# merijn-23/magr-ray-tracer

Measured on AMD Instinct MI355X. Metric: Mrays/sec + extend-kernel HBM GB/s, sponza 1080p 256spp, higher is better.
Workload: dtype f32

## Files before the change

### include/rt355.h

```cpp
#ifndef RT355_H
#define RT355_H
#include "rt355_types.h"

#ifdef __cplusplus
extern "C" {
#endif

#define RT_OK            0
#define RT_E_INVALID    (-1)
#define RT_E_DEVICE     (-2)
#define RT_E_NOMEM      (-3)
#define RT_E_UNSUPPORTED (-4)

#define RT_SHADING_SIMPLE       0
#define RT_SHADING_NEE          1
#define RT_SAMPLING_HEMISPHERE  0
#define RT_SAMPLING_COSINE      1
#define RT_ACCEL_BVH2           0
#define RT_ACCEL_BVH4           1

typedef struct RtCtx RtCtx;

typedef struct RtConfig {
    int32_t width, height;
// ... 21 lines not shown
    uint64_t shadow_rays;
    uint64_t frames;
    uint64_t extend_node_issues, extend_leaf_issues, connect_node_issues, connect_leaf_issues;
    uint64_t extend_loop_node_events, extend_loop_leaf_events, connect_loop_node_events, connect_loop_leaf_events;
} RtCounters;

typedef struct RtStageTimes {
    double  generate_ms, extend_ms, shade_ms, compact_ms, connect_ms, accumulate_ms;
    int64_t generate_launches, extend_launches, shade_launches, compact_launches, connect_launches, accumulate_launches;
} RtStageTimes;

typedef struct RtKernelInfo {
    int32_t layout;
    int32_t persist, persist4;
    int32_t stack_entries;
    int32_t persist_grid, persist_grid_connect, shade_grid;
    int32_t n_blas;
} RtKernelInfo;

const char* rt_last_error(void);
int rt_device_count(void);
int rt_kernel_info(RtCtx* ctx, RtKernelInfo* out);
int rt_builtins(RtCtx* ctx);

int rt_create(const RtConfig* cfg, RtCtx** out);
int rt_destroy(RtCtx* ctx);

int rt_upload_scene(RtCtx* ctx,
                    const RtPrimitive* prims, int32_t nPrims,
                    const RtMaterial* mats, int32_t nMats,
                    const RtFloat4* textures, int32_t nTexels,
                    const uint32_t* lights, int32_t nLights,
                    const void* bvhNodes, int32_t nNodes,
                    const uint32_t* primIdx, int32_t nIdx,
                    const RtTLASNode* tlas, int32_t nTlas,
                    const RtBVHInstance* blas, int32_t nBlas);

int rt_upload_scene_bvh2(RtCtx* ctx,
                         const RtPrimitive* prims, int32_t nPrims, const RtMaterial* mats, int32_t nMats,
                         const RtFloat4* textures, int32_t nTexels, const uint32_t* lights, int32_t nLights,
                         const RtBVHNode2* bvhNodes, int32_t nNodes, const uint32_t* primIdx, int32_t nIdx,
                         const RtTLASNode* tlas, int32_t nTlas, const RtBVHInstance* blas, int32_t nBlas);

int rt_validate_scene(int32_t accel,
                      const RtPrimitive* prims, int32_t nPrims, const RtMaterial* mats, int32_t nMats,
                      const RtFloat4* textures, int32_t nTexels, const uint32_t* lights, int32_t nLights,
// ... 151 lines not shown
```

### magr_ray_tracer_amd/_lib.py

```python
import ctypes as C
import os

import numpy as np

_PKG = os.path.dirname(os.path.abspath(__file__))

f4 = np.dtype((np.float32, 4))
Ray = np.dtype([("O", f4), ("D", f4), ("rD", f4), ("N", f4), ("I", f4), ("intensity", f4), ("t", "<f4"),
                ("primIdx", "<i4"), ("bounces", "<i4"), ("pixelIdx", "<i4"), ("inside", "u1"), ("lastSpecular", "u1"),
                ("_pad0", "u1", 2), ("u", "<f4"), ("v", "<f4"), ("_pad1", "<u4")], align=False)
ShadowRay = np.dtype([("I", f4), ("L", f4), ("Nl", f4), ("intensity", f4), ("BRDF", f4), ("lightIdx", "<i4"),
                      ("pixelIdx", "<i4"), ("dotNL", "<f4"), ("dist", "<f4")])
Material = np.dtype([("color", f4), ("absorption", f4), ("specular", "<f4"), ("n1", "<f4"), ("n2", "<f4"),
                     ("isDielectric", "u1"), ("_pad0", "u1", 3), ("texIdx", "<i4"), ("texW", "<i4"), ("texH", "<i4"),
                     ("isLight", "u1"), ("_pad1", "u1", 3), ("emittance", f4)])
Primitive = np.dtype([("v0", f4), ("v1", f4), ("v2", f4), ("N", f4), ("centroid", f4), ("uv0", "<f4", 2), ("uv1", "<f4", 2),
                      ("uv2", "<f4", 2), ("_padt", "<f4", 2), ("objType", "<i4"), ("matIdx", "<i4"), ("area", "<f4"),
                      ("_pad", "<u4")])
Camera = np.dtype([("type", "<i4"), ("fov", "<f4"), ("aperture", "<f4"), ("focalLength", "<f4"), ("forward", f4),
                   ("right", f4), ("up", f4), ("origin", f4), ("horizontal", f4), ("vertical", f4), ("topLeft", f4)])
Settings = np.dtype([("numPrimitives", "<i4"), ("numLights", "<i4"), ("tracerType", "<i4"), ("frames", "<i4"),
                     ("antiAliasing", "<i4"), ("numInRays", "<i4"), ("numOutRays", "<i4"), ("shadowRays", "<i4"),
                     ("renderBVH", "<i4"), ("focalLength", "<f4")])
BVHNode2 = np.dtype([("aabbMin", f4), ("aabbMax", f4), ("first", "<u4"), ("count", "<u4"), ("_pad", "<u4", 2)])
# ... 43 lines not shown


def builtins_value(name):
    try:
        return BUILTINS[name]
    except (KeyError, TypeError):
        raise ValueError(f"builtins must be None, 'ieee' or 'reference', not {name!r}") from None


RT_OK, RT_E_INVALID, RT_E_DEVICE, RT_E_NOMEM, RT_E_UNSUPPORTED = 0, -1, -2, -3, -4
SCENE_ARRAYS = {"prims": 0, "bvh": 1, "tlas": 2, "instances": 3, "pairs": 4, "triRecs": 5, "shadeRecs": 6, "lightRecs": 7,
                "tlasPairs": 8, "tlasPairsP": 9, "instRecs": 10}
SCENE_ARRAYS_BVH4 = {"quads": 11, "rootEntry": 12, "bvh2Kept": 13}
UpdateStats = np.dtype([("gpu_ms", "<f8"), ("prims", "<i4"), ("nodes", "<i4"), ("tlas_nodes", "<i4"), ("tlas_depth", "<i4"),
                        ("reconfigured", "<i4"), ("reserved", "<i4", 3)])
assert UpdateStats.itemsize == 40
REBUILD_SAH, REBUILD_LBVH, REBUILD_SBVH = 0, 1, 2
RebuildStats = np.dtype([(n, "<f8") for n in ("gpu_ms", "wall_ms", "stage_ms", "build_ms", "derive_ms", "tlas_ms", "commit_ms")] +
                        [(n, "<i4") for n in ("prims", "blas_built", "nodes", "n_idx", "max_depth", "tlas_nodes", "tlas_depth", "reconfigured")] +
                        [("spatial_splits", "<i4"), ("prims_clipped", "<i4")])
assert RebuildStats.itemsize == 96

DEVICE_SYMBOLS = [
    "rt_last_error", "rt_device_count", "rt_kernel_info", "rt_builtins", "rt_create", "rt_destroy", "rt_upload_scene", "rt_share_scene", "rt_set_seeds", "rt_seed_default",
    "rt_get_seeds", "rt_bind_accum", "rt_accum_device_ptr", "rt_stream", "rt_reset", "rt_render", "rt_synchronize", "rt_focus",
    "rt_read_accum", "rt_write_accum", "rt_postproc", "rt_read_counters", "rt_reset_counters", "rt_read_stage_times", "rt_reset_stage_times", "rt_set_profile",
    "rt_stage_begin_frame", "rt_stage_generate", "rt_stage_extend", "rt_stage_shade", "rt_stage_connect",
    "rt_debug_get_rays", "rt_debug_set_rays", "rt_debug_get_shadow", "rt_debug_enable_steps", "rt_debug_get_steps", "rt_debug_math",
    "rt_debug_math_sweep", "rt_debug_math_mode", "rt_debug_math_sweep_mode", "rt_validate_scene", "rt_build_bvh2", "rt_build_bvh2_sah", "rt_debug_sah_phases", "rt_build_bvh2_sbvh", "rt_debug_sbvh_phases", "rt_update_scene", "rt_group_update_scene", "rt_debug_get_scene_array",
    "rt_rebuild_scene", "rt_group_rebuild_scene", "rt_blas_ranges", "rt_debug_rebuild_allocations",
    "rt_build_bvh4", "rt_upload_scene_bvh2", "rt_group_upload_scene_bvh2",
    "rt_group_create", "rt_group_destroy", "rt_group_lanes", "rt_group_concurrency", "rt_group_lane", "rt_group_frames", "rt_group_upload_scene", "rt_group_share_scene",
    "rt_group_seed", "rt_group_reset", "rt_group_render", "rt_group_synchronize", "rt_group_sum", "rt_group_read_accum", "rt_group_focus",
    "rt_group_postproc"]
HOST_SYMBOLS = [
    "rth_last_error", "rth_scene_create", "rth_scene_destroy", "rth_add_material", "rth_add_texture", "rth_load_texture", "rth_add_sphere",
    "rth_add_plane", "rth_add_triangle", "rth_add_quad", "rth_add_triangles", "rth_build_blas", "rth_build_bvh4",
    "rth_build_tlas", "rth_bvh4_from_nodes", "rth_set_instance_transform", "rth_primitives", "rth_materials", "rth_textures", "rth_lights",
    "rth_bvh2_nodes", "rth_bvh4_nodes", "rth_prim_idx", "rth_tlas_nodes", "rth_blas_nodes", "rth_bvh_stats", "rth_camera",
    "rth_renderer_create", "rth_renderer_destroy", "rth_renderer_init", "rth_renderer_set_camera", "rth_renderer_tick",
    "rth_renderer_read", "rth_renderer_camera", "rth_seed_stream", "rth_load_model", "rth_save_png",
    "rth_set_build_threads", "rth_renderer_save_frame", "rth_renderer_camera_move", "rth_renderer_camera_mouse", "rth_renderer_camera_zoom", "rth_renderer_frames", "rth_renderer_set_lanes", "rth_renderer_set_builtins", "rth_renderer_builtins",
    "rth_build_blas_lbvh", "rth_build_bvh2_lbvh", "rth_lbvh_stats", "rth_set_primitives", "rth_refit",
    "rth_build_blas_sah_gpu", "rth_build_bvh2_sah", "rth_build_blas_sbvh_gpu", "rth_build_bvh2_sbvh", "rth_rebuild", "rth_blas_ranges",
    "rth_build_bvh4_gpu", "rth_build_bvh4_levels"]

_dev = None
# ... 18 lines not shown

def device_lib(variant=None):
    global _dev
    if variant:
        if variant not in _variants:
            keep, _dev = _dev, None
            try:
                _variants[variant] = _bind_device(_load(f"librt355_{variant}.so", local=True))
            finally:
                _dev = keep
        return _variants[variant]
    if _dev is None:
        _dev = _bind_device(_load("librt355.so"))
    return _dev


def _bind_device(lib):
    if True:
        vp, i32, i64 = C.c_void_p, C.c_int32, C.c_int64
        lib.rt_last_error.restype = C.c_char_p
        lib.rt_create.argtypes = [vp, C.POINTER(vp)]
        lib.rt_kernel_info.argtypes = [vp, vp]
        lib.rt_builtins.argtypes = [vp]
        lib.rt_destroy.argtypes = [vp]
        lib.rt_upload_scene.argtypes = [vp, vp, i32, vp, i32, vp, i32, vp, i32, vp, i32, vp, i32, vp, i32, vp, i32]
        lib.rt_upload_scene_bvh2.argtypes = lib.rt_upload_scene.argtypes
        lib.rt_group_upload_scene_bvh2.argtypes = lib.rt_upload_scene.argtypes
        lib.rt_build_bvh4.argtypes = [i32, vp, i32, i32, vp, i32, vp, vp]
        lib.rt_share_scene.argtypes = [vp, vp]
        lib.rt_set_seeds.argtypes = [vp, vp, i64]
        lib.rt_seed_default.argtypes = [vp]
        lib.rt_get_seeds.argtypes = [vp, vp, i64]
        lib.rt_bind_accum.argtypes = [vp, vp]
        lib.rt_accum_device_ptr.argtypes = [vp]
        lib.rt_accum_device_ptr.restype = vp
        lib.rt_stream.argtypes = [vp]
        lib.rt_stream.restype = vp
        lib.rt_reset.argtypes = [vp]
        lib.rt_render.argtypes = [vp, vp, vp, i32]
        lib.rt_synchronize.argtypes = [vp]
        lib.rt_focus.argtypes = [vp, i32, i32, vp, C.POINTER(C.c_float)]
        lib.rt_read_accum.argtypes = [vp, vp]
        lib.rt_read_counters.argtypes = [vp, vp]
        lib.rt_write_accum.argtypes = [vp, vp]
        lib.rt_postproc.argtypes = [vp, i32, C.c_float, C.c_float, C.c_float, vp, vp]
        lib.rt_reset_counters.argtypes = [vp]
# ... 130 lines not shown
```

### magr_ray_tracer_amd/csrc/rt355.hip

```cpp
#include <hip/hip_runtime.h>
#include <hip/hip_ext.h>
#include <algorithm>
#include <chrono>
#include <cstdio>
#include <cmath>
#include <cstdlib>
#include <cstring>
#include <memory>
#include <atomic>
#include <string>
#include <vector>
#include "../../include/rt355.h"
#include "rt355_kernels.h"
#include "scene_dev.h"

using namespace rt355dev;
using namespace scenedev;

static constexpr int kAdmitAnySgpr = 6, kAdmit96Sgpr = 7;
static constexpr int kFitSeven = 22, kBackupWords = 10, kSpillCap = kFitSeven - kBackupWords;
static thread_local std::string g_err;
int rt355_set_error(int code, const char* msg) { g_err = msg; return code; }

struct RtCtx {
    RtConfig cfg{};
    hipStream_t stream = nullptr;
    hipStream_t home = nullptr;
    bool queued = true;
    DevScene sc{};
    DevQueues q{};
    DevVariant var{};
    int nPix = 0, firstPixel = 0, gridMax = 0;
    bool sceneLoaded = false, ownAccum = true;
    std::shared_ptr<SceneBag> scene;
    uint64_t sceneGen = 0;
    bool singleBlas = false;
    std::vector<void*> queueAllocs;
    float* dFocus = nullptr;
    RtRay* dRayIO = nullptr;
    uint64_t frames = 0, primaryRays = 0;
    struct Ev { hipEvent_t a, b; int stage; };
    std::vector<Ev> evPool; size_t evUsed = 0;
// ... 58 lines not shown
static bool bvh4_tlas_trav(const RtCtx* c) { return c->trav == TRAV_BVH4_TLAS || c->trav == TRAV_BVH4_TLAS_SPILL; }
static bool tlas_trav(const RtCtx* c) { return c->trav == TRAV_TLAS || c->trav == TRAV_TLAS_SPILL || bvh4_tlas_trav(c); }

extern "C" const char* rt_last_error(void) { return g_err.c_str(); }
extern "C" int rt_device_count(void) { int n = 0; if (hipGetDeviceCount(&n) != hipSuccess) return 0; return n; }
static int sync_scene_config(RtCtx* ctx);
extern "C" int rt_builtins(RtCtx* ctx)
{
    if (!ctx) return fail(RT_E_INVALID, "rt_builtins: null context");
    return ctx->cfg.builtins;
}
extern "C" int rt_kernel_info(RtCtx* ctx, RtKernelInfo* out)
{
    if (!ctx || !out) return fail(RT_E_INVALID, "rt_kernel_info: null argument");
    if (!ctx->sceneLoaded) return fail(RT_E_INVALID, "rt_kernel_info: no scene uploaded");
    if (const int rc = sync_scene_config(ctx)) return rc;
    const int persist = ctx->trav <= TRAV_TLAS_SPILL ? ctx->trav : 0;
    const int persist4 = ctx->trav == TRAV_BVH4 ? 1 : (ctx->trav == TRAV_BVH4_TLAS ? 2 : (ctx->trav == TRAV_BVH4_TLAS_SPILL ? 3 : 0));
    *out = RtKernelInfo{ ctx->layout, persist, persist4, spill_trav(ctx) ? ctx->spillCap : ctx->stackEntries, ctx->persistGrid, ctx->persistGridConnect,
                         ctx->shadeGrid, ctx->sc.nBlas };
    return RT_OK;
}

static void free_bag(std::vector<void*>& bag) { for (void* p : bag) (void)hipFree(p); bag.clear(); }

static void scene_release(RtCtx* ctx)
{
    if (!ctx->scene) return;
    auto& h = ctx->scene->holders;
    h.erase(std::remove(h.begin(), h.end(), ctx), h.end());
    ctx->scene.reset();
}
static void scene_hold(RtCtx* ctx, const std::shared_ptr<SceneBag>& bag)
{
    scene_release(ctx);
    ctx->scene = bag;
    bag->holders.push_back(ctx);
}
int SceneBag::wait_holders() const
{
    for (const RtCtx* h : holders) {
        HIPCHK(hipStreamSynchronize(h->stream));
        if (h->home != h->stream) HIPCHK(hipStreamSynchronize(h->home));
    }
    return RT_OK;
}

static size_t stack_bytes(const RtCtx* c) { return (size_t)c->stackEntries * kBlock * sizeof(uint32_t); }
static int tlas_stack_entries(const RtCtx* c) { return c->stackEntries + c->tlasDepth + 1; }
static int tlas_lds_entries(const RtCtx* c) { return spill_trav(c) ? c->spillCap : tlas_stack_entries(c); }
static size_t tlas_column_bytes(int entries) { return (size_t)(entries + kBackupWords) * kBlock * sizeof(uint32_t); }
static size_t tlas_stack_bytes(const RtCtx* c) { return tlas_column_bytes(tlas_lds_entries(c)); }
static inline dim3 grid_for(int n) { return dim3((unsigned)std::max(1, (n + kBlock - 1) / kBlock)); }

using PersistKernel = void (*)(DevScene, DevQueues, int, int, int, PersistTune);
using NestedKernel = void (*)(DevScene, DevQueues, int, int);
struct TraceLaunch {
    PersistKernel persist = nullptr;
    NestedKernel nested = nullptr;
    dim3 grid;
    size_t lds = 0;
    PersistTune tune{};
};
static TraceLaunch trace_launch(const RtCtx* c, int stage, int bounce, bool steps, int rays)
{
    TraceLaunch L;
    L.grid = grid_for(rays);
    L.lds = stack_bytes(c);
    const bool connect = stage == ST_CONNECT;
    const bool bvh4 = c->cfg.accel == RT_ACCEL_BVH4, l1 = c->layout == 1;
    switch (c->trav) {
    case TRAV_NESTED:
        if (connect) L.nested = bvh4 ? (l1 ? k_connect<RT_ACCEL_BVH4, 1> : k_connect<RT_ACCEL_BVH4, 0>) : (l1 ? k_connect<RT_ACCEL_BVH2, 1> : k_connect<RT_ACCEL_BVH2, 0>);
        else L.nested = bvh4 ? (l1 ? k_extend<RT_ACCEL_BVH4, 1> : k_extend<RT_ACCEL_BVH4, 0>) : (l1 ? k_extend<RT_ACCEL_BVH2, 1> : k_extend<RT_ACCEL_BVH2, 0>);
        break;
    case TRAV_BVH2:
        L.tune = connect ? c->tuneConnect : c->tune;
        if (connect) { L.persist = k_trace_persist<true>; L.grid = dim3(c->persistGridConnect); }
        else if (bounce > 0 || c->cfg.extend_variant == 3) { L.persist = steps ? k_trace_persist<false, false, true> : k_trace_persist<false>; L.grid = dim3(c->persistGrid); }
        else if (c->cfg.extend_variant == 5) L.nested = k_extend<RT_ACCEL_BVH2, 1>;
        else L.persist = c->coherent ? k_trace_persist<false, true> : (steps ? k_trace_persist<false, false, true> : k_trace_persist<false>);
        break;
    case TRAV_BVH4:
        L.tune = connect ? c->tuneConnect : c->tune4;
        L.persist = connect ? k_trace_persist4<true> : k_trace_persist4<false>;
        if (connect || bounce > 0) L.grid = dim3(connect ? c->persistGridConnect : c->persistGrid);
        break;
    case TRAV_TLAS:
    case TRAV_TLAS_SPILL: {
        const bool spill = c->trav == TRAV_TLAS_SPILL;
        L.lds = tlas_stack_bytes(c);
        if (connect) {
            L.tune = c->tuneConnect;
            L.persist = spill ? k_trace_persist_tlas<true, false, true> : k_trace_persist_tlas<true>;
            L.grid = dim3(c->persistGridConnect);
            break;
        }
        L.tune = c->tune;
        if (bounce > 0 || spill) L.grid = dim3(c->persistGrid);
        const bool coh = c->coherent && (bounce == 0 || c->coherent == 2) && (c->tune.flat || !spill);
        if (steps) L.persist = spill ? k_trace_persist_tlas<false, true, true> : k_trace_persist_tlas<false, true>;
        else if (coh) L.persist = spill ? k_trace_persist_tlas<false, false, true, true> : k_trace_persist_tlas<false, false, false, true>;
        else L.persist = spill ? k_trace_persist_tlas<false, false, true> : k_trace_persist_tlas<false>;
        break;
    }
    case TRAV_BVH4_TLAS:
    case TRAV_BVH4_TLAS_SPILL: {
        const bool spill = c->trav == TRAV_BVH4_TLAS_SPILL;
        L.lds = tlas_stack_bytes(c);
        if (connect) {
            L.tune = c->tuneConnect;
            L.persist = spill ? k_trace_persist4_tlas<true, false, true> : k_trace_persist4_tlas<true>;
            L.grid = dim3(c->persistGridConnect);
            break;
        }
        L.tune = c->tune4;
        if (bounce > 0 || spill) L.grid = dim3(c->persistGrid);
        if (steps) L.persist = spill ? k_trace_persist4_tlas<false, true, true> : k_trace_persist4_tlas<false, true>;
        else L.persist = spill ? k_trace_persist4_tlas<false, false, true> : k_trace_persist4_tlas<false>;
        break;
    }
    }
    return L;
}

static constexpr size_t kEvRing = 4096;
static void ev_account(RtCtx* c, RtCtx::Ev& e)
{
    float ms = 0;
    if (hipEventElapsedTime(&ms, e.a, e.b) != hipSuccess) { (void)hipEventSynchronize(e.b); (void)hipEventElapsedTime(&ms, e.a, e.b); }
    switch (e.stage) {
    case ST_GENERATE: c->times.generate_ms += ms; c->times.generate_launches++; break;
    case ST_EXTEND:   c->times.extend_ms += ms; c->times.extend_launches++; break;
    case ST_SHADE:    c->times.shade_ms += ms; c->times.shade_launches++; break;
    case ST_COMPACT:  c->times.compact_ms += ms; c->times.compact_launches++; break;
    case ST_CONNECT:  c->times.connect_ms += ms; c->times.connect_launches++; break;
    case ST_ACCUM:    c->times.accumulate_ms += ms; c->times.accumulate_launches++; break;
    }
    e.stage = -1;
}
static void ev_init(RtCtx* c)
{
    if (!c->cfg.profile || !c->evPool.empty()) return;
    c->evPool.resize(kEvRing);
    for (auto& e : c->evPool) { (void)hipEventCreate(&e.a); (void)hipEventCreate(&e.b); e.stage = -1; }
}
// ... 160 lines not shown
        if ((tlas_stack_entries(ctx) > kFitSeven || forceSpill || !fits) && canSpill) ctx->trav = TRAV_BVH4_TLAS_SPILL;
        else if (!fits) ctx->trav = TRAV_NESTED;
    }
    ctx->coherent = getenv("RT355_COHERENT") ? atoi(getenv("RT355_COHERENT")) : 1;

    ctx->tune = PersistTune{ 112, 24, 6, 8, 0 }; ctx->tuneConnect = PersistTune{ 128, 32, 6, 16, 0 }; ctx->tune4 = PersistTune{ 64, 20, 6, 8, 0 };
    if (ctx->cfg.persist_blocks_per_cu > 0) {
        ctx->tune.leafK = 16;
    } else {
        ctx->tune.fixedChunks = ctx->tuneConnect.fixedChunks = ctx->tune4.fixedChunks = 1;
    }
    int tuneBlocks = 0;
    if (const char* t = getenv("RT355_TUNE")) {
        int a = 0, b = 0, c = 0, l = 0, d = 0;
        int k = sscanf(t, "%d,%d,%d,%d,%d", &a, &b, &c, &l, &d);
        if (k >= 4 && a > 0 && b > 0 && b <= 64 && c > 0 && l > 0 && l <= 64) ctx->tune = ctx->tuneConnect = ctx->tune4 = PersistTune{ a, b, c, l, 0 };
        if (k == 5 && d > 0) tuneBlocks = d;
    }
    if (const char* t = getenv("RT355_FIXED_CHUNKS")) { int a = 0, b = 0; if (sscanf(t, "%d,%d", &a, &b) == 2) { ctx->tune.fixedChunks = ctx->tune4.fixedChunks = a; ctx->tuneConnect.fixedChunks = b; } }
    if (const char* t = getenv("RT355_TUNE_CONNECT")) {
        int a = 0, b = 0, c = 0, l = 0;
        if (sscanf(t, "%d,%d,%d,%d", &a, &b, &c, &l) == 4 && a > 0 && b > 0 && b <= 64 && c > 0 && l > 0 && l <= 64) ctx->tuneConnect = PersistTune{ a, b, c, l, 0 };
    }
    if (tlas_trav(ctx)) {
        ctx->tune.flat = ctx->tune4.flat = 1; ctx->tuneConnect.flat = 0;
        if (const char* t = getenv("RT355_TLAS_FLAT")) { int a = 0, b = 0; if (sscanf(t, "%d,%d", &a, &b) == 2) { ctx->tune.flat = ctx->tune4.flat = a; ctx->tuneConnect.flat = b; } }
    }
    {
        static std::atomic<int> serial{ 0 };
        if (ctx->xcdFirst < 0) ctx->xcdFirst = serial.fetch_add(1) & 7;
        int rays = 1024;
        if (const char* t = getenv("RT355_XCD_RAYS")) rays = std::max(0, atoi(t));
        ctx->tune.xcdRays = ctx->tuneConnect.xcdRays = ctx->tune4.xcdRays = rays;
        ctx->tune.xcdFirst = ctx->tuneConnect.xcdFirst = ctx->tune4.xcdFirst = ctx->xcdFirst;
        int thin = 16;
        if (const char* t = getenv("RT355_THIN")) thin = std::min(64, std::max(0, atoi(t)));
        ctx->tune.thin = ctx->tuneConnect.thin = ctx->tune4.thin = thin;
    }

    if (persistent(ctx)) {
        int perCU = 0; hipDeviceProp_t prop;
        HIPCHK(hipGetDeviceProperties(&prop, ctx->cfg.device));
        const TraceLaunch L = trace_launch(ctx, ST_EXTEND, 1, false, ctx->nPix);
        HIPCHK(hipOccupancyMaxActiveBlocksPerMultiprocessor(&perCU, L.persist, kBlock, L.lds));
        const int mp = prop.multiProcessorCount;
        int perCUc = perCU;
        if (bvh4_tlas_trav(ctx)) {
            const TraceLaunch C = trace_launch(ctx, ST_CONNECT, 0, false, ctx->nPix);
            HIPCHK(hipOccupancyMaxActiveBlocksPerMultiprocessor(&perCUc, C.persist, kBlock, C.lds));
        }
        ctx->persistGrid = std::min(ctx->gridMax, std::max(1, std::min(perCU, kAdmit96Sgpr)) * mp);
        ctx->persistGridConnect = std::min(ctx->gridMax, std::max(1, std::min(perCUc, kAdmitAnySgpr)) * mp);
        if (ctx->cfg.persist_blocks_per_cu > 0) {
            ctx->persistGrid = std::min(ctx->persistGrid, std::min(ctx->gridMax, std::min(ctx->cfg.persist_blocks_per_cu, std::max(1, perCU)) * mp));
            ctx->persistGridConnect = std::min(ctx->persistGridConnect, std::min(ctx->gridMax, std::min(ctx->cfg.persist_blocks_per_cu, std::max(1, perCUc)) * mp));
        }
        if (tuneBlocks > 0) {
            ctx->persistGrid = std::min(ctx->gridMax, std::min(tuneBlocks, std::max(1, perCU)) * mp);
            ctx->persistGridConnect = std::min(ctx->gridMax, std::min(tuneBlocks, std::max(1, perCUc)) * mp);
        }
        if (const char* t = getenv("RT355_CONNECT_BLOCKS")) { const int d = atoi(t); if (d > 0) ctx->persistGridConnect = std::min(ctx->gridMax, std::min(d, std::max(1, perCUc)) * mp); }
    }
    ctx->q.spill = nullptr; ctx->q.spillStride = 0; ctx->q.stackCap = 0;
    ctx->q.tlasLdsEntries = tlas_trav(ctx) ? (uint32_t)tlas_lds_entries(ctx) : 0u;
    if (spill_trav(ctx)) {
        const size_t stride = (size_t)std::max(ctx->persistGrid, ctx->persistGridConnect) * kBlock;
        const size_t words = stride * (size_t)(tlas_stack_entries(ctx) - ctx->spillCap);
        if (words > ctx->spillWords) {
            if (ctx->dSpill) (void)hipFree(ctx->dSpill);
            ctx->dSpill = nullptr; ctx->spillWords = 0;
            if (hipMalloc((void**)&ctx->dSpill, words * sizeof(uint32_t)) != hipSuccess) return fail(RT_E_NOMEM, "hipMalloc of the spill stacks (%zu bytes) failed", words * sizeof(uint32_t));
            ctx->spillWords = words;
        }
        ctx->q.spill = ctx->dSpill; ctx->q.spillStride = (uint32_t)stride; ctx->q.stackCap = (uint32_t)ctx->spillCap;
    }
    return RT_OK;
}

static int adopt_scene(RtCtx* ctx)
{
    const SceneBag& b = *ctx->scene;
    const SceneArrays& a = b.sc;
    auto f4 = [](const RtFloat4* p) { return (const float4*)p; };
    ctx->sc = DevScene{ a.prims, a.mats, f4(a.tex), a.lights, a.bvh2, a.bvh4, a.primIdx, a.tlas, a.blas, f4(a.pairs), f4(a.triRecs), a.rootEntry, f4(a.shadeRecs),
// ... 911 lines not shown
```

### magr_ray_tracer_amd/csrc/rt355_kernels.h

```cpp
#pragma once
#include <hip/hip_runtime.h>
#include <stdint.h>
#include "../../include/rt355_types.h"

namespace rt355dev {

#define RT_FORCEINLINE __device__ __forceinline__
static constexpr int   kBlock = 256;
static constexpr float kEps = RT_EPSILON;
static constexpr float kFar = RT_REALLYFAR;
static constexpr float kPi = 3.14159274101257f;
static constexpr float kInvPi = 0.31830987334251f;

struct DevScene {
    const RtPrimitive*   prims;
    const RtMaterial*    mats;
    const float4*        tex;
    const uint32_t*      lights;
    const RtBVHNode2*    bvh2;
    const RtBVHNode4*    bvh4;
    const uint32_t*      primIdx;
    const RtTLASNode*    tlas;
    const RtBVHInstance* blas;
    const float4*        pairs;
// ... 669 lines not shown
        TRay r;
        r.ox = O.x; r.oy = O.y; r.oz = O.z; r.dx = D.x; r.dy = D.y; r.dz = D.z;
        r.rx = 1.0f / D.x; r.ry = 1.0f / D.y; r.rz = 1.0f / D.z;
        r.t = kFar; r.prim = -1; r.u = 0.0f; r.v = 0.0f;
        int steps = traverse_tlas<ACCEL, LAYOUT, false>(sc, r, stk, wc);
        rays = 1;
        q.hit[i] = mk4(r.t, __int_as_float(r.prim), r.u, r.v);
        if (q.steps) q.steps[i] = steps;
        if (renderBVH) q.accum[q.firstPixel + i] = splat((float)(uint32_t)steps / 255.f);
    }
    flush_counters(q.ctrExtend, rays, wc, stk);
}

#ifdef RT355_TAIL_PROBE
static constexpr int kTpWaves = 8192;
__device__ unsigned long long g_tp[9][kTpWaves][4];
#endif
struct PersistTune {
    int chunk, refill, inner, leafK;
    int fixedChunks;
    int flat = 0;
    int xcdRays = 0, xcdFirst = 0;
    int thin = 0;
};

RT_FORCEINLINE int xcd_pack(int n, int xcdRays, int xcdFirst, int& waves)
{
    const int wpb = kBlock / 64, wave = threadIdx.x >> 6;
    waves = gridDim.x * wpb;
    if (xcdRays <= 0 || (gridDim.x & 7u) != 0u) return blockIdx.x * wpb + wave;
    const int perXcd = (int)(gridDim.x >> 3) * kBlock;
    int nx = min(8, max(1, (n + xcdRays - 1) / xcdRays));
    while (nx < 8 && (long long)nx * perXcd < (long long)n) nx++;
    if (nx == 8) return blockIdx.x * wpb + wave;
    const int xcd = (int)(blockIdx.x + 8u - (uint32_t)xcdFirst) & 7;
    waves = (int)(gridDim.x >> 3) * nx * wpb;
    if (xcd >= nx) return -1;
    return ((int)(blockIdx.x >> 3) * nx + xcd) * wpb + wave;
}

struct SparseMap { int first, stride, per; };
RT_FORCEINLINE SparseMap sparse_map(int n, const PersistTune& t, int waveId)
{
    SparseMap m = { waveId, (int)gridDim.x * (kBlock / 64), 64 };
    if (t.xcdRays <= 0 && t.thin <= 0) return m;
    m.first = xcd_pack(n, t.xcdRays, t.xcdFirst, m.stride);
// ... 86 lines not shown
        if (next >= end) {
            int c = 0;
            if (t.fixedChunks) { round++; c = round * nWaves * t.chunk + waveId * t.chunk; }
            else {
                if (lane == 0) c = atomicAdd(w.cursor, t.chunk);
                c = __shfl(c, 0, 64) + nWaves * t.chunk;
            }
            next = c; end = min(c + t.chunk, w.n);
            if (c >= w.n) { exhausted = true; next = end = 0; }
#ifdef RT355_TAIL_PROBE
            if (exhausted) tpDry = wall_clock64();
#endif
        }
        if (next < end) {
            const int i = next + __popcll(idleMask & ((1ull << lane) - 1ull));
            if (idle && i < end) idx = i;
            dealt += (uint32_t)min(nIdle, end - next);
            next = min(next + nIdle, end);
        }
        return true;
    }
};

template <bool OCC, bool COH, bool BVH4 = false>
RT_FORCEINLINE void trace_short_queue(const DevScene& sc, const DevQueues& q, int b0, const QueueWindow& w, int renderBVH, const OneInstance& one,
                                      uint32_t* stk, int waveId, int lane, const PersistTune& tune)
{
    WorkCtr wc = { 0, 0, 0, 0 };
    uint32_t rays = 0;
    const int idx = short_queue_slot<OCC>(q, b0, w.n, tune, waveId, lane);
    if (idx < w.n) {
        TRay r;
        queue_ray<OCC>(r, q, b0, w.first, idx, &one);
        rays = 1; wc.inst = 1;
        const int st = BVH4 ? traverse_bvh4_packed<OCC>(sc, r, one.root, stk, wc)
                     : COH ? traverse_bvh2_packed_coherent(sc, r, one.root, stk, wc) : traverse_bvh2_packed<OCC>(sc, r, one.root, stk, wc);
        store_result<OCC, true>(q, w.first, idx, r, st, st == -1, renderBVH);
    }
    flush_counters(OCC ? q.ctrConnect : q.ctrExtend, rays, wc, stk);
}


template <bool OCC, bool COH = false, bool STEPS = false>
__global__ __launch_bounds__(kBlock) void k_trace_persist(DevScene sc, DevQueues q, int b0, int b1, int renderBVH, PersistTune tune)
{
    const int kInner = tune.inner, kLeafK = tune.leafK;
    extern __shared__ uint32_t stk[];
    const int lane = threadIdx.x & 63;
    const QueueWindow w = queue_window<OCC>(q, b0, b1);
    const OneInstance one = one_instance(sc);

    WorkCtr wc = { 0, 0, 0, 0 };
    uint32_t rays = 0;
    uint32_t wRays = 0, wNode = 0, wPrim = 0, wNodeIss = 0, wLeafIss = 0;
    TRay r; r.t = 0; r.prim = -1; r.u = r.v = 0; r.ox = r.oy = r.oz = r.dx = r.dy = r.dz = r.rx = r.ry = r.rz = 0;
    uint32_t cur = 0, sp = 0;
    int slot = -1, steps = 0;
    float tLight = 0;
    const int nWaves = gridDim.x * (kBlock / 64), waveId = blockIdx.x * (kBlock / 64) + (threadIdx.x >> 6);
#ifdef RT355_TAIL_PROBE
    const unsigned long long tp0 = wall_clock64();
#define TAIL_PROBE_EXIT(tpDry) if (lane == 0 && waveId < kTpWaves) { unsigned long long* p = g_tp[OCC ? 8 : b0][waveId]; p[0] = tp0; p[1] = tpDry; p[2] = wall_clock64(); p[3] = rays; }
#endif
    if (w.n <= nWaves * 64) {
        trace_short_queue<OCC, COH>(sc, q, b0, w, renderBVH, one, stk, waveId, lane, tune);
#ifdef RT355_TAIL_PROBE
        TAIL_PROBE_EXIT(0ull)
#endif
        return;
    }
    ChunkDealer deal(waveId, tune.chunk, w.n);
    for (;;) {
        int idx;
        if (!deal.refill(slot < 0, idx, wRays, w, tune, nWaves, waveId, lane)) break;
        if (idx >= 0) { queue_ray<OCC>(r, q, b0, w.first, idx, &one); tLight = r.t; cur = one.root; sp = 0; steps = 0; slot = idx; }
#pragma unroll 1
        for (int it = 0; it < kInner; it++) {
            const bool act = slot >= 0, atLeaf = act && (cur & kLeafBit) != 0u;
            const unsigned long long lm = __ballot(atLeaf), im = __ballot(act && !atLeaf);
            if ((lm | im) == 0ull) break;
            const bool doLeaf = im == 0ull || __popcll(lm) >= kLeafK;
            bool done = false, occluded = false;
            if (!doLeaf) { wNode += (uint32_t)__popcll(im); if (STEPS) wNodeIss++; }
            if (doLeaf) {
                wPrim += (uint32_t)__popcll(lm); if (STEPS) wLeafIss++;
                if (atLeaf) {
                    const uint32_t first = cur & 0x00ffffffu, count = (cur >> 24) & 0x7fu;
                    test_tri_packed(sc, first, r);
                    if (OCC && r.t < tLight) { done = true; occluded = true; }
                    else if (count > 1) cur = kLeafBit | ((count - 1) << 24) | (first + 1);
                    else if (sp == 0) done = true;
                    else cur = STK(--sp);
                }
            } else if (act && !atLeaf) {
                const float4* p = sc.pairs + (size_t)cur * 4;
                const float4 q0 = p[0], q1 = p[1], q2 = p[2], q3 = p[3];
                uint32_t e1 = __float_as_uint(q3.x), e2 = __float_as_uint(q3.y);
                if (OCC) {
                    float x1, x2;
                    const bool h1 = slab_any(r, mk4(q0.x, q0.y, q0.z, 0.0f), mk4(q0.w, q1.x, q1.y, 0.0f), x1);
                    const bool h2 = slab_any(r, mk4(q1.z, q1.w, q2.x, 0.0f), mk4(q2.y, q2.z, q2.w, 0.0f), x2);
                    if (h1 && h2) { const bool firstIs2 = x2 > x1; cur = firstIs2 ? e2 : e1; STK(sp) = firstIs2 ? e1 : e2; sp++; }
                    else if (h1 || h2) cur = h1 ? e1 : e2;
                    else if (sp == 0) done = true;
                    else cur = STK(--sp);
                } else {
                    float d1 = slab(r, mk4(q0.x, q0.y, q0.z, 0.0f), mk4(q0.w, q1.x, q1.y, 0.0f));
                    float d2 = slab(r, mk4(q1.z, q1.w, q2.x, 0.0f), mk4(q2.y, q2.z, q2.w, 0.0f));
                    if (d1 > d2) { float d = d1; d1 = d2; d2 = d; uint32_t e = e1; e1 = e2; e2 = e; }
                    if (d1 >= tLight) {
                        if (sp == 0) done = true;
                        else cur = STK(--sp);
                    } else {
                        if (STEPS) steps++;
                        cur = e1;
                        if (d2 < tLight) { STK(sp) = e2; sp++; if (STEPS) steps++; }
                    }
                }
            }
            if (done) { store_result<OCC, STEPS>(q, w.first, slot, r, steps, occluded, renderBVH); slot = -1; }
        }
    }
#ifdef RT355_TAIL_PROBE
    TAIL_PROBE_EXIT(deal.tpDry)
#endif
    if (lane == 0) { rays = wRays; wc.inst = wRays; wc.node = wNode; wc.prim = wPrim; if (STEPS) { wc.nodeIss = wNodeIss; wc.leafIss = wLeafIss; wc.evNode = wNode; wc.evPrim = wPrim; } }
    flush_counters(OCC ? q.ctrConnect : q.ctrExtend, rays, wc, stk);
}

static constexpr uint32_t kTagTlas = 0x40000000u, kTagInst = 0x60000000u, kTagMask = 0xe0000000u, kIdMask = 0x1fffffffu;
RT_FORCEINLINE bool slab_both(const TRay& r, float4 bmin, float4 bmax, float& tminOut, float& tmaxOut)
{
    float tx1 = (bmin.x - r.ox) * r.rx, tx2 = (bmax.x - r.ox) * r.rx;
    float tmin = fminf(tx1, tx2), tmax = fmaxf(tx1, tx2);
    float ty1 = (bmin.y - r.oy) * r.ry, ty2 = (bmax.y - r.oy) * r.ry;
    tmin = fmaxf(tmin, fminf(ty1, ty2)); tmax = fminf(tmax, fmaxf(ty1, ty2));
    float tz1 = (bmin.z - r.oz) * r.rz, tz2 = (bmax.z - r.oz) * r.rz;
    tmin = fmaxf(tmin, fminf(tz1, tz2)); tmax = fminf(tmax, fmaxf(tz1, tz2));
    tminOut = tmin; tmaxOut = tmax;
    return tmax >= tmin && tmin < r.t && tmax > 0;
}
// ... 995 lines not shown
```

### magr_ray_tracer_amd/renderer.py

```python
import ctypes as C

import numpy as np

from . import _lib


class RtError(RuntimeError):
    code = None


def _update_args(prims, first, instances):
    p = None if prims is None else np.ascontiguousarray(prims, dtype=_lib.Primitive)
    b = None if instances is None else np.ascontiguousarray(instances, dtype=_lib.BVHInstance)
    st = np.zeros((), dtype=_lib.UpdateStats)
    args = (_lib.ptr(p) if p is not None and len(p) else None, int(first), 0 if p is None else len(p),
            _lib.ptr(b) if b is not None else None, 0 if b is None else len(b), _lib.ptr(st))
    return args, (p, b), st


def _update_dict(st):
    return {"gpu_ms": float(st["gpu_ms"]), "prims": int(st["prims"]), "nodes": int(st["nodes"]), "tlas_nodes": int(st["tlas_nodes"]),
            "tlas_depth": int(st["tlas_depth"]), "reconfigured": bool(st["reconfigured"])}


# ... 97 lines not shown
            e.code = rc
            raise e
        return _rebuild_dict(st)

    def rebuild_allocations(self):
        n = C.c_int64(0)
        self._chk(self._lib.rt_debug_rebuild_allocations(self._h, C.byref(n)))
        return n.value

    def scene_array(self, name):
        which = _lib.SCENE_ARRAYS[name] if name in _lib.SCENE_ARRAYS else _lib.SCENE_ARRAYS_BVH4[name]
        n = C.c_int64(0)
        self._chk(self._lib.rt_debug_get_scene_array(self._h, which, None, 0, C.byref(n)))
        out = np.zeros(n.value, dtype=np.uint8)
        if n.value:
            self._chk(self._lib.rt_debug_get_scene_array(self._h, which, _lib.ptr(out), n.value, C.byref(n)))
        return out

    def kernel_info(self):
        k = np.zeros((), dtype=_lib.KernelInfo)
        self._chk(self._lib.rt_kernel_info(self._h, k.ctypes.data_as(C.c_void_p)))
        return {n: int(k[n]) for n in k.dtype.names}

    @property
    def builtins(self):
        rc = self._lib.rt_builtins(self._h)
        if rc < 0:
            self._chk(rc)
        return int(rc)

    def extend_kernel_name(self):
        k = self.kernel_info()
        if k["persist4"] == 3:
            return "k_trace_persist4_tlas<false, false, true> (LDS stack of %d entries per lane, deeper entries in global memory)" % k["stack_entries"]
        if k["persist4"] == 2:
            return "k_trace_persist4_tlas<false> (bounce 0: its one-ray-per-lane branch)"
        if k["persist4"]:
            return "k_trace_persist4<false>"
        if k["persist"] == 3:
            return "k_trace_persist_tlas<false, false, true> (LDS stack of %d entries per lane, deeper entries in global memory)" % k["stack_entries"]
        if k["persist"] == 2:
            return "k_trace_persist_tlas<false> (bounce 0: its one-ray-per-lane branch)"
        if k["persist"]:
            return "k_trace_persist<false> (bounce 0: <false, true>, node records of wave-uniform visits through the scalar cache)"
        return "k_extend<%s, %d>" % ("RT_ACCEL_BVH4" if self.accel == _lib.ACCEL_BVH4 else "RT_ACCEL_BVH2", k["layout"])

# ... 315 lines not shown
```

Baseline: 988.5.

## Cache top BVH levels in LDS for persistent BVH2 traversal

Each persistent BVH2 trace block now copies the top few levels of the BVH (up to 6, i.e. 63 nodes) from global memory into LDS once. Fresh rays then descend those levels in lockstep from LDS before falling back to the normal global-memory traversal loop. The goal is to cut repeated global loads of the hottest top nodes. In exchange the kernel uses more LDS per block, which could lower occupancy. An auto-tuner lowers the level count until the persistent grid size matches the configuration without the cache.

```diff
diff --git a/include/rt355.h b/include/rt355.h
--- a/include/rt355.h
+++ b/include/rt355.h
@@ -67,6 +67,7 @@
 int rt_device_count(void);
 int rt_kernel_info(RtCtx* ctx, RtKernelInfo* out);
 int rt_builtins(RtCtx* ctx);
+int rt_top_levels(RtCtx* ctx, int32_t* extend, int32_t* connect);
 
 int rt_create(const RtConfig* cfg, RtCtx** out);
 int rt_destroy(RtCtx* ctx);
diff --git a/magr_ray_tracer_amd/_lib.py b/magr_ray_tracer_amd/_lib.py
--- a/magr_ray_tracer_amd/_lib.py
+++ b/magr_ray_tracer_amd/_lib.py
@@ -89,7 +89,7 @@
 assert RebuildStats.itemsize == 96
 
 DEVICE_SYMBOLS = [
-    "rt_last_error", "rt_device_count", "rt_kernel_info", "rt_builtins", "rt_create", "rt_destroy", "rt_upload_scene", "rt_share_scene", "rt_set_seeds", "rt_seed_default",
+    "rt_last_error", "rt_device_count", "rt_kernel_info", "rt_builtins", "rt_top_levels", "rt_create", "rt_destroy", "rt_upload_scene", "rt_share_scene", "rt_set_seeds", "rt_seed_default",
     "rt_get_seeds", "rt_bind_accum", "rt_accum_device_ptr", "rt_stream", "rt_reset", "rt_render", "rt_synchronize", "rt_focus",
     "rt_read_accum", "rt_write_accum", "rt_postproc", "rt_read_counters", "rt_reset_counters", "rt_read_stage_times", "rt_reset_stage_times", "rt_set_profile",
     "rt_stage_begin_frame", "rt_stage_generate", "rt_stage_extend", "rt_stage_shade", "rt_stage_connect",
@@ -154,6 +154,7 @@
         lib.rt_create.argtypes = [vp, C.POINTER(vp)]
         lib.rt_kernel_info.argtypes = [vp, vp]
         lib.rt_builtins.argtypes = [vp]
+        lib.rt_top_levels.argtypes = [vp, C.POINTER(i32), C.POINTER(i32)]
         lib.rt_destroy.argtypes = [vp]
         lib.rt_upload_scene.argtypes = [vp, vp, i32, vp, i32, vp, i32, vp, i32, vp, i32, vp, i32, vp, i32, vp, i32]
         lib.rt_upload_scene_bvh2.argtypes = lib.rt_upload_scene.argtypes
diff --git a/magr_ray_tracer_amd/csrc/rt355.hip b/magr_ray_tracer_amd/csrc/rt355.hip
--- a/magr_ray_tracer_amd/csrc/rt355.hip
+++ b/magr_ray_tracer_amd/csrc/rt355.hip
@@ -18,6 +18,7 @@
 using namespace scenedev;
 
 static constexpr int kAdmitAnySgpr = 6, kAdmit96Sgpr = 7;
+static constexpr int kTopLevelsExtend = 6, kTopLevelsConnect = 6;
 static constexpr int kFitSeven = 22, kBackupWords = 10, kSpillCap = kFitSeven - kBackupWords;
 static thread_local std::string g_err;
 int rt355_set_error(int code, const char* msg) { g_err = msg; return code; }
@@ -122,6 +123,15 @@
     return RT_OK;
 }
 
+extern "C" int rt_top_levels(RtCtx* ctx, int32_t* extend, int32_t* connect)
+{
+    if (!ctx || !extend || !connect) return fail(RT_E_INVALID, "rt_top_levels: null argument");
+    if (!ctx->sceneLoaded) return fail(RT_E_INVALID, "rt_top_levels: no scene uploaded");
+    if (const int rc = sync_scene_config(ctx)) return rc;
+    *extend = ctx->tune.topLevels; *connect = ctx->tuneConnect.topLevels;
+    return RT_OK;
+}
+
 static void free_bag(std::vector<void*>& bag) { for (void* p : bag) (void)hipFree(p); bag.clear(); }
 
 static void scene_release(RtCtx* ctx)
@@ -147,6 +157,7 @@
 }
 
 static size_t stack_bytes(const RtCtx* c) { return (size_t)c->stackEntries * kBlock * sizeof(uint32_t); }
+static size_t top_bytes(int levels) { return levels > 0 ? (((size_t)1 << levels) - 1) * 4 * sizeof(float4) : 0; }
 static int tlas_stack_entries(const RtCtx* c) { return c->stackEntries + c->tlasDepth + 1; }
 static int tlas_lds_entries(const RtCtx* c) { return spill_trav(c) ? c->spillCap : tlas_stack_entries(c); }
 static size_t tlas_column_bytes(int entries) { return (size_t)(entries + kBackupWords) * kBlock * sizeof(uint32_t); }
@@ -162,13 +173,14 @@
     size_t lds = 0;
     PersistTune tune{};
 };
-static TraceLaunch trace_launch(const RtCtx* c, int stage, int bounce, bool steps, int rays)
+static TraceLaunch trace_launch(const RtCtx* c, int stage, int bounce, bool steps, int rays, int topLevels = -1 )
 {
     TraceLaunch L;
     L.grid = grid_for(rays);
     L.lds = stack_bytes(c);
     const bool connect = stage == ST_CONNECT;
     const bool bvh4 = c->cfg.accel == RT_ACCEL_BVH4, l1 = c->layout == 1;
+    bool top = false;
     switch (c->trav) {
     case TRAV_NESTED:
         if (connect) L.nested = bvh4 ? (l1 ? k_connect<RT_ACCEL_BVH4, 1> : k_connect<RT_ACCEL_BVH4, 0>) : (l1 ? k_connect<RT_ACCEL_BVH2, 1> : k_connect<RT_ACCEL_BVH2, 0>);
@@ -176,10 +188,17 @@
         break;
     case TRAV_BVH2:
         L.tune = connect ? c->tuneConnect : c->tune;
-        if (connect) { L.persist = k_trace_persist<true>; L.grid = dim3(c->persistGridConnect); }
-        else if (bounce > 0 || c->cfg.extend_variant == 3) { L.persist = steps ? k_trace_persist<false, false, true> : k_trace_persist<false>; L.grid = dim3(c->persistGrid); }
+        if (topLevels >= 0) L.tune.topLevels = topLevels;
+        if (connect) { top = L.tune.topLevels > 0; L.persist = top ? k_trace_persist<true, false, false, true> : k_trace_persist<true>; L.grid = dim3(c->persistGridConnect); }
+        else if (bounce > 0 || c->cfg.extend_variant == 3) {
+            top = L.tune.topLevels > 0;
+            if (top) L.persist = steps ? k_trace_persist<false, false, true, true> : k_trace_persist<false, false, false, true>;
+            else L.persist = steps ? k_trace_persist<false, false, true> : k_trace_persist<false>;
+            L.grid = dim3(c->persistGrid);
+        }
         else if (c->cfg.extend_variant == 5) L.nested = k_extend<RT_ACCEL_BVH2, 1>;
         else L.persist = c->coherent ? k_trace_persist<false, true> : (steps ? k_trace_persist<false, false, true> : k_trace_persist<false>);
+        if (top) { L.tune.topBase = c->stackEntries * kBlock; L.lds += top_bytes(L.tune.topLevels); }
         break;
     case TRAV_BVH4:
         L.tune = connect ? c->tuneConnect : c->tune4;
@@ -222,6 +241,23 @@
     }
     }
     return L;
+}
+
+static int persist_query(const RtCtx* c, int stage, int topLevels, int* perCU)
+{
+    const TraceLaunch L = trace_launch(c, stage, stage == ST_CONNECT ? 0 : 1, false, c->nPix, topLevels);
+    HIPCHK(hipOccupancyMaxActiveBlocksPerMultiprocessor(perCU, L.persist, kBlock, L.lds));
+    return RT_OK;
+}
+static int persist_blocks(const RtCtx* c, int stage, int perCU, int tuneBlocks)
+{
+    const bool connect = stage == ST_CONNECT;
+    const int fit = std::max(1, perCU);
+    int g = std::max(1, std::min(perCU, connect ? kAdmitAnySgpr : kAdmit96Sgpr));
+    if (c->cfg.persist_blocks_per_cu > 0) g = std::min(g, std::min(c->cfg.persist_blocks_per_cu, fit));
+    if (tuneBlocks > 0) g = std::min(tuneBlocks, fit);
+    if (connect) if (const char* t = getenv("RT355_CONNECT_BLOCKS")) { const int d = atoi(t); if (d > 0) g = std::min(d, fit); }
+    return g;
 }
 
 static constexpr size_t kEvRing = 4096;
@@ -428,6 +464,18 @@
         int a = 0, b = 0, c = 0, l = 0;
         if (sscanf(t, "%d,%d,%d,%d", &a, &b, &c, &l) == 4 && a > 0 && b > 0 && b <= 64 && c > 0 && l > 0 && l <= 64) ctx->tuneConnect = PersistTune{ a, b, c, l, 0 };
     }
+    ctx->tune.topLevels = ctx->tuneConnect.topLevels = 0;
+    bool topAuto = false;
+    if (ctx->trav == TRAV_BVH2) {
+        ctx->tune.topLevels = kTopLevelsExtend; ctx->tuneConnect.topLevels = kTopLevelsConnect;
+        topAuto = true;
+        if (const char* t = getenv("RT355_TOP_LEVELS")) {
+            int a = 0, b = 0;
+            const int k = sscanf(t, "%d,%d", &a, &b);
+            if (k == 1) b = a;
+            if (k >= 1 && a >= 0 && a <= kTopMaxLevels && b >= 0 && b <= kTopMaxLevels) { ctx->tune.topLevels = a; ctx->tuneConnect.topLevels = b; topAuto = false; }
+        }
+    }
     if (tlas_trav(ctx)) {
         ctx->tune.flat = ctx->tune4.flat = 1; ctx->tuneConnect.flat = 0;
         if (const char* t = getenv("RT355_TLAS_FLAT")) { int a = 0, b = 0; if (sscanf(t, "%d,%d", &a, &b) == 2) { ctx->tune.flat = ctx->tune4.flat = a; ctx->tuneConnect.flat = b; } }
@@ -447,25 +495,23 @@
     if (persistent(ctx)) {
         int perCU = 0; hipDeviceProp_t prop;
         HIPCHK(hipGetDeviceProperties(&prop, ctx->cfg.device));
-        const TraceLaunch L = trace_launch(ctx, ST_EXTEND, 1, false, ctx->nPix);
-        HIPCHK(hipOccupancyMaxActiveBlocksPerMultiprocessor(&perCU, L.persist, kBlock, L.lds));
-        const int mp = prop.multiProcessorCount;
+        for (PersistTune* t : { &ctx->tune, &ctx->tuneConnect }) if (stack_bytes(ctx) + top_bytes(t->topLevels) > prop.sharedMemPerBlock) t->topLevels = 0;
+        if (topAuto) for (int stage : { ST_EXTEND, ST_CONNECT }) {
+            PersistTune& t = stage == ST_CONNECT ? ctx->tuneConnect : ctx->tune;
+            int q = 0, lv = t.topLevels;
+            if (const int rc = persist_query(ctx, stage, 0, &q)) return rc;
+            const int base = persist_blocks(ctx, stage, q, tuneBlocks);
+            for (; lv > 0; lv--) {
+                if (const int rc = persist_query(ctx, stage, lv, &q)) return rc;
+                if (persist_blocks(ctx, stage, q, tuneBlocks) == base) break;
+            }
+            t.topLevels = lv;
+        }
+        if (const int rc = persist_query(ctx, ST_EXTEND, -1, &perCU)) return rc;
         int perCUc = perCU;
-        if (bvh4_tlas_trav(ctx)) {
-            const TraceLaunch C = trace_launch(ctx, ST_CONNECT, 0, false, ctx->nPix);
-            HIPCHK(hipOccupancyMaxActiveBlocksPerMultiprocessor(&perCUc, C.persist, kBlock, C.lds));
-        }
-        ctx->persistGrid = std::min(ctx->gridMax, std::max(1, std::min(perCU, kAdmit96Sgpr)) * mp);
-        ctx->persistGridConnect = std::min(ctx->gridMax, std::max(1, std::min(perCUc, kAdmitAnySgpr)) * mp);
-        if (ctx->cfg.persist_blocks_per_cu > 0) {
-            ctx->persistGrid = std::min(ctx->persistGrid, std::min(ctx->gridMax, std::min(ctx->cfg.persist_blocks_per_cu, std::max(1, perCU)) * mp));
-            ctx->persistGridConnect = std::min(ctx->persistGridConnect, std::min(ctx->gridMax, std::min(ctx->cfg.persist_blocks_per_cu, std::max(1, perCUc)) * mp));
-        }
-        if (tuneBlocks > 0) {
-            ctx->persistGrid = std::min(ctx->gridMax, std::min(tuneBlocks, std::max(1, perCU)) * mp);
-            ctx->persistGridConnect = std::min(ctx->gridMax, std::min(tuneBlocks, std::max(1, perCUc)) * mp);
-        }
-        if (const char* t = getenv("RT355_CONNECT_BLOCKS")) { const int d = atoi(t); if (d > 0) ctx->persistGridConnect = std::min(ctx->gridMax, std::min(d, std::max(1, perCUc)) * mp); }
+        if (bvh4_tlas_trav(ctx) || ctx->tuneConnect.topLevels > 0) { if (const int rc = persist_query(ctx, ST_CONNECT, -1, &perCUc)) return rc; }
+        ctx->persistGrid = std::min(ctx->gridMax, persist_blocks(ctx, ST_EXTEND, perCU, tuneBlocks) * prop.multiProcessorCount);
+        ctx->persistGridConnect = std::min(ctx->gridMax, persist_blocks(ctx, ST_CONNECT, perCUc, tuneBlocks) * prop.multiProcessorCount);
     }
     ctx->q.spill = nullptr; ctx->q.spillStride = 0; ctx->q.stackCap = 0;
     ctx->q.tlasLdsEntries = tlas_trav(ctx) ? (uint32_t)tlas_lds_entries(ctx) : 0u;
diff --git a/magr_ray_tracer_amd/csrc/rt355_kernels.h b/magr_ray_tracer_amd/csrc/rt355_kernels.h
--- a/magr_ray_tracer_amd/csrc/rt355_kernels.h
+++ b/magr_ray_tracer_amd/csrc/rt355_kernels.h
@@ -715,6 +715,7 @@
     int flat = 0;
     int xcdRays = 0, xcdFirst = 0;
     int thin = 0;
+    int topLevels = 0, topBase = 0;
 };
 
 RT_FORCEINLINE int xcd_pack(int n, int xcdRays, int xcdFirst, int& waves)
@@ -847,6 +848,78 @@
     }
 };
 
+template <bool OCC, bool STEPS>
+RT_FORCEINLINE int node_event(const TRay& r, float tLight, float4 q0, float4 q1, float4 q2, float4 q3, uint32_t* stk, uint32_t& cur, uint32_t& sp, int& steps, bool& done)
+{
+    uint32_t e1 = __float_as_uint(q3.x), e2 = __float_as_uint(q3.y);
+    int child = 0;
+    if (OCC) {
+        float x1, x2;
+        const bool h1 = slab_any(r, mk4(q0.x, q0.y, q0.z, 0.0f), mk4(q0.w, q1.x, q1.y, 0.0f), x1);
+        const bool h2 = slab_any(r, mk4(q1.z, q1.w, q2.x, 0.0f), mk4(q2.y, q2.z, q2.w, 0.0f), x2);
+        if (h1 && h2) { const bool firstIs2 = x2 > x1; cur = firstIs2 ? e2 : e1; STK(sp) = firstIs2 ? e1 : e2; sp++; child = firstIs2 ? 2 : 1; }
+        else if (h1 || h2) { cur = h1 ? e1 : e2; child = h1 ? 1 : 2; }
+        else if (sp == 0) done = true;
+        else cur = STK(--sp);
+    } else {
+        float d1 = slab(r, mk4(q0.x, q0.y, q0.z, 0.0f), mk4(q0.w, q1.x, q1.y, 0.0f));
+        float d2 = slab(r, mk4(q1.z, q1.w, q2.x, 0.0f), mk4(q2.y, q2.z, q2.w, 0.0f));
+        const bool swap = d1 > d2;
+        if (swap) { float d = d1; d1 = d2; d2 = d; uint32_t e = e1; e1 = e2; e2 = e; }
+        if (d1 >= tLight) {
+            if (sp == 0) done = true;
+            else cur = STK(--sp);
+        } else {
+            if (STEPS) steps++;
+            cur = e1; child = swap ? 2 : 1;
+            if (d2 < tLight) { STK(sp) = e2; sp++; if (STEPS) steps++; }
+        }
+    }
+    return child;
+}
+
+static constexpr int kTopMaxLevels = 6;
+RT_FORCEINLINE void fill_top(const DevScene& sc, uint32_t root, float4* top, int levels)
+{
+    const float4 absent = mk4(__uint_as_float(kLeafBit), __uint_as_float(kLeafBit), 0.0f, 0.0f);
+    for (int l = 0; l < levels; l++) {
+        const int n = 1 << l, t = (int)threadIdx.x;
+        if (t < n) {
+            const int s = n - 1 + t;
+            uint32_t e = root;
+            if (l > 0) { const float4 up = top[((s - 1) >> 1) * 4 + 3]; e = __float_as_uint((s & 1) ? up.x : up.y); }
+            float4 q0 = splat(0.0f), q1 = q0, q2 = q0, q3 = absent;
+            if (!(e & kLeafBit)) { const float4* p = sc.pairs + (size_t)e * 4; q0 = p[0]; q1 = p[1]; q2 = p[2]; q3 = p[3]; }
+            float4* o = top + s * 4;
+            o[0] = q0; o[1] = q1; o[2] = q2; o[3] = q3;
+        }
+        __syncthreads();
+    }
+}
+
+template <bool OCC, bool STEPS>
+RT_FORCEINLINE void top_descent(const DevQueues& q, const QueueWindow& w, int renderBVH, const float4* top, int levels, bool fresh, const TRay& r, float tLight,
+                                uint32_t* stk, uint32_t& cur, uint32_t& sp, int& steps, int& slot, uint32_t& wNode, uint32_t& wNodeIss)
+{
+    const uint32_t nSlots = (1u << levels) - 1u;
+    uint32_t ts = 0;
+    bool in = fresh && nSlots != 0u && !(cur & kLeafBit);
+    for (;;) {
+        const unsigned long long m = __ballot(in);
+        if (m == 0ull) break;
+        wNode += (uint32_t)__popcll(m); if (STEPS) wNodeIss++;
+        if (in) {
+            const float4* p = top + ts * 4;
+            const float4 q0 = p[0], q1 = p[1], q2 = p[2], q3 = p[3];
+            bool done = false;
+            const int child = node_event<OCC, STEPS>(r, tLight, q0, q1, q2, q3, stk, cur, sp, steps, done);
+            if (done) { store_result<OCC, STEPS>(q, w.first, slot, r, steps, false, renderBVH); slot = -1; }
+            ts = 2u * ts + (uint32_t)child;
+            in = child != 0 && ts < nSlots && !(cur & kLeafBit);
+        }
+    }
+}
+
 template <bool OCC, bool COH, bool BVH4 = false>
 RT_FORCEINLINE void trace_short_queue(const DevScene& sc, const DevQueues& q, int b0, const QueueWindow& w, int renderBVH, const OneInstance& one,
                                       uint32_t* stk, int waveId, int lane, const PersistTune& tune)
@@ -866,7 +939,7 @@
 }
 
 
-template <bool OCC, bool COH = false, bool STEPS = false>
+template <bool OCC, bool COH = false, bool STEPS = false, bool TOP = false>
 __global__ __launch_bounds__(kBlock) void k_trace_persist(DevScene sc, DevQueues q, int b0, int b1, int renderBVH, PersistTune tune)
 {
     const int kInner = tune.inner, kLeafK = tune.leafK;
@@ -894,11 +967,14 @@
 #endif
         return;
     }
+    float4* const top = reinterpret_cast<float4*>(stk + tune.topBase);
+    if (TOP) fill_top(sc, one.root, top, tune.topLevels);
     ChunkDealer deal(waveId, tune.chunk, w.n);
     for (;;) {
         int idx;
         if (!deal.refill(slot < 0, idx, wRays, w, tune, nWaves, waveId, lane)) break;
         if (idx >= 0) { queue_ray<OCC>(r, q, b0, w.first, idx, &one); tLight = r.t; cur = one.root; sp = 0; steps = 0; slot = idx; }
+        if (TOP) top_descent<OCC, STEPS>(q, w, renderBVH, top, tune.topLevels, idx >= 0, r, tLight, stk, cur, sp, steps, slot, wNode, wNodeIss);
 #pragma unroll 1
         for (int it = 0; it < kInner; it++) {
             const bool act = slot >= 0, atLeaf = act && (cur & kLeafBit) != 0u;
@@ -920,28 +996,7 @@
             } else if (act && !atLeaf) {
                 const float4* p = sc.pairs + (size_t)cur * 4;
                 const float4 q0 = p[0], q1 = p[1], q2 = p[2], q3 = p[3];
-                uint32_t e1 = __float_as_uint(q3.x), e2 = __float_as_uint(q3.y);
-                if (OCC) {
-                    float x1, x2;
-                    const bool h1 = slab_any(r, mk4(q0.x, q0.y, q0.z, 0.0f), mk4(q0.w, q1.x, q1.y, 0.0f), x1);
-                    const bool h2 = slab_any(r, mk4(q1.z, q1.w, q2.x, 0.0f), mk4(q2.y, q2.z, q2.w, 0.0f), x2);
-                    if (h1 && h2) { const bool firstIs2 = x2 > x1; cur = firstIs2 ? e2 : e1; STK(sp) = firstIs2 ? e1 : e2; sp++; }
-                    else if (h1 || h2) cur = h1 ? e1 : e2;
-                    else if (sp == 0) done = true;
-                    else cur = STK(--sp);
-                } else {
-                    float d1 = slab(r, mk4(q0.x, q0.y, q0.z, 0.0f), mk4(q0.w, q1.x, q1.y, 0.0f));
-                    float d2 = slab(r, mk4(q1.z, q1.w, q2.x, 0.0f), mk4(q2.y, q2.z, q2.w, 0.0f));
-                    if (d1 > d2) { float d = d1; d1 = d2; d2 = d; uint32_t e = e1; e1 = e2; e2 = e; }
-                    if (d1 >= tLight) {
-                        if (sp == 0) done = true;
-                        else cur = STK(--sp);
-                    } else {
-                        if (STEPS) steps++;
-                        cur = e1;
-                        if (d2 < tLight) { STK(sp) = e2; sp++; if (STEPS) steps++; }
-                    }
-                }
+                node_event<OCC, STEPS>(r, tLight, q0, q1, q2, q3, stk, cur, sp, steps, done);
             }
             if (done) { store_result<OCC, STEPS>(q, w.first, slot, r, steps, occluded, renderBVH); slot = -1; }
         }
diff --git a/magr_ray_tracer_amd/renderer.py b/magr_ray_tracer_amd/renderer.py
--- a/magr_ray_tracer_amd/renderer.py
+++ b/magr_ray_tracer_amd/renderer.py
@@ -143,6 +143,11 @@
         self._chk(self._lib.rt_kernel_info(self._h, k.ctypes.data_as(C.c_void_p)))
         return {n: int(k[n]) for n in k.dtype.names}
 
+    def top_levels(self):
+        e, c = C.c_int32(0), C.c_int32(0)
+        self._chk(self._lib.rt_top_levels(self._h, C.byref(e), C.byref(c)))
+        return int(e.value), int(c.value)
+
     @property
     def builtins(self):
         rc = self._lib.rt_builtins(self._h)
```

New measurement: 1005, median of 6. +1.7%, better.
